# rll/rllab

Measured on NVIDIA H100. Metric: env-steps/sec (full iteration: rollout + process_samples + VPG update), higher is better.
Workload: dtype f32

## Files before the change

### rllab_b200/csrc/tile_gram.cuh

```cuda
#pragma once
#include "update_common.cuh"

namespace b200rl {

struct TileDist {
  float ls_new[3], inv_std[3], ls_old[3], inv_std_old[3], Mmu[3], var_new[3], var_new2[3], var_old[3];
  float sum_ls_new, sum_ls_old, half_log2pi_A;
};

template <class N, int MODE>
__device__ __forceinline__ void tile_dist_init(TileDist& D, const float* log_std_params, const UpdArgs& a) {
  constexpr int A = N::A;
  D.sum_ls_new = 0.f;
  D.sum_ls_old = 0.f;
#pragma unroll
  for (int k = 0; k < A; ++k) {
    D.ls_new[k] = clamp_log_std(log_std_params[k], a.log_min_std);
    const float sd = expf(D.ls_new[k]);
    D.inv_std[k] = 1.0f / sd;
    D.var_new[k] = sd * sd;
    D.var_new2[k] = 2.0f * sd * sd + 1e-8f;
    D.Mmu[k] = 2.0f / D.var_new2[k];
    D.ls_old[k] = (MODE == MODE_FVP) ? D.ls_new[k] : a.old_log_std[k];
    const float so = expf(D.ls_old[k]);
    D.inv_std_old[k] = 1.0f / so;
    D.var_old[k] = so * so;
    D.sum_ls_new += D.ls_new[k];
    D.sum_ls_old += D.ls_old[k];
  }
  D.half_log2pi_A = 0.5f * (float)A * 1.8378770664093453f;
}

template <class N, int RX, int RH1, int RH2, int RD1, int RD2, int RDM, int LD, bool PACKED = false>
struct TileGram {
  static constexpr int O = N::O, H = 32, A = N::A, TILE = 128;
  static constexpr int OQ = (O + 3) / 4;
  static_assert(N::H1 == 32 && N::H2 == 32 && A <= 3, "32-wide layers, act_dim <= 3");
  double accW1[4][4];
  double accB[OQ + 1];
  double accA;
  double accT;

  __device__ __forceinline__ void init() {
#pragma unroll
    for (int r = 0; r < 4; ++r)
#pragma unroll
      for (int c = 0; c < 4; ++c) accW1[r][c] = 0.0;
#pragma unroll
    for (int k = 0; k <= OQ; ++k) accB[k] = 0.0;
    accA = 0.0;
    accT = 0.0;
  }

  __device__ __forceinline__ void accumulate_a(const float* stage, int tid) {
    const int w1_tile = tid & 63, kh = tid >> 6;
    const int ti = w1_tile >> 3, tj = w1_tile & 7;
    const float* U = stage + (RH1 + ti) * LD + kh * 64;
    const float* V = stage + (RD2 + tj) * LD + kh * 64;
    if constexpr (PACKED) {
      float2 acc[4][4];
#pragma unroll
      for (int r = 0; r < 4; ++r)
#pragma unroll
        for (int c = 0; c < 4; ++c) acc[r][c] = make_float2(0.f, 0.f);
#pragma unroll 2
      for (int k = 0; k < 64; k += 4) {
        float4 u[4], v[4];
#pragma unroll
        for (int r = 0; r < 4; ++r) u[r] = *reinterpret_cast<const float4*>(U + r * 8 * LD + k);
#pragma unroll
        for (int c = 0; c < 4; ++c) v[c] = *reinterpret_cast<const float4*>(V + c * 8 * LD + k);
        gram_4x4(u, v, acc);
      }
#pragma unroll
      for (int r = 0; r < 4; ++r)
#pragma unroll
        for (int c = 0; c < 4; ++c) accW1[r][c] += (double)(acc[r][c].x + acc[r][c].y);
    } else {
      float acc[4][4];
#pragma unroll
      for (int r = 0; r < 4; ++r)
#pragma unroll
        for (int c = 0; c < 4; ++c) acc[r][c] = 0.f;
#pragma unroll 4
      for (int k = 0; k < 64; k += 4) {
        float4 u[4], v[4];
#pragma unroll
        for (int r = 0; r < 4; ++r) u[r] = *reinterpret_cast<const float4*>(U + r * 8 * LD + k);
#pragma unroll
        for (int c = 0; c < 4; ++c) v[c] = *reinterpret_cast<const float4*>(V + c * 8 * LD + k);
#pragma unroll
        for (int r = 0; r < 4; ++r)
#pragma unroll
          for (int c = 0; c < 4; ++c) {
            acc[r][c] = fmaf(u[r].x, v[c].x, acc[r][c]);
            acc[r][c] = fmaf(u[r].y, v[c].y, acc[r][c]);
            acc[r][c] = fmaf(u[r].z, v[c].z, acc[r][c]);
            acc[r][c] = fmaf(u[r].w, v[c].w, acc[r][c]);
          }
      }
#pragma unroll
      for (int r = 0; r < 4; ++r)
#pragma unroll
        for (int c = 0; c < 4; ++c) accW1[r][c] += (double)acc[r][c];
    }
    const int lane = tid & 31, wq = tid >> 5;
    if (wq < A) {
      const float* Hh = stage + (RH2 + lane) * LD;
      const float* M = stage + (RDM + wq) * LD;
      float s0 = 0.f, s1 = 0.f;
#pragma unroll 4
      for (int k = 0; k < TILE; k += 4) {
        const float4 hv = *reinterpret_cast<const float4*>(Hh + k);
        const float4 m = *reinterpret_cast<const float4*>(M + k);
        s0 = fmaf(hv.x, m.x, s0); s1 = fmaf(hv.y, m.y, s1);
        s0 = fmaf(hv.z, m.z, s0); s1 = fmaf(hv.w, m.w, s1);
      }
      accA += (double)(s0 + s1);
    } else if (wq == 3) {
      const float* Dr = stage + (RD2 + lane) * LD;
      float s0 = 0.f;
#pragma unroll 4
      for (int k = 0; k < TILE; k += 4) {
        const float4 d = *reinterpret_cast<const float4*>(Dr + k);
        s0 += (d.x + d.y) + (d.z + d.w);
      }
      accA += (double)s0;
    }
    if (tid < 2 * A) {
      const float* Dr = stage + (RDM + tid) * LD;
      float s0 = 0.f;
#pragma unroll 4
      for (int k = 0; k < TILE; k += 4) {
        const float4 d = *reinterpret_cast<const float4*>(Dr + k);
        s0 += (d.x + d.y) + (d.z + d.w);
      }
      accT += (double)s0;
    }
  }

  __device__ __forceinline__ void accumulate_b(const float* stage, int tid) {
    const int lane = tid & 31, wq = tid >> 5;
    const float* Dr = stage + (RD1 + lane) * LD;
    float sa[OQ + 1];
#pragma unroll
    for (int i = 0; i <= OQ; ++i) sa[i] = 0.f;
#pragma unroll 4
    for (int k = 0; k < TILE; k += 4) {
      const float4 d = *reinterpret_cast<const float4*>(Dr + k);
#pragma unroll
      for (int i = 0; i < OQ; ++i) {
        const int o = wq + 4 * i;
        if (o < O) {
          const float4 xv = *reinterpret_cast<const float4*>(stage + (RX + o) * LD + k);
          sa[i] = fmaf(xv.x, d.x, sa[i]); sa[i] = fmaf(xv.y, d.y, sa[i]);
          sa[i] = fmaf(xv.z, d.z, sa[i]); sa[i] = fmaf(xv.w, d.w, sa[i]);
        }
      }
      if (wq == 3) sa[OQ] += (d.x + d.y) + (d.z + d.w);
    }
#pragma unroll
    for (int i = 0; i <= OQ; ++i) accB[i] += (double)sa[i];
  }

  __device__ __forceinline__ void write(double* out, double* scr, int tid) {
    write(out, scr, tid, [] { __syncthreads(); });
  }
  template <class Sync>
  __device__ __forceinline__ void write(double* out, double* scr, int tid, Sync sync) {
    const int w1_tile = tid & 63, kh = tid >> 6;
    const int ti = w1_tile >> 3, tj = w1_tile & 7;
#pragma unroll
    for (int r = 0; r < 4; ++r)
#pragma unroll
      for (int c = 0; c < 4; ++c) scr[(kh * 64 + w1_tile) * 16 + r * 4 + c] = accW1[r][c];
    sync();
    if (tid < 64) {
#pragma unroll
      for (int r = 0; r < 4; ++r)
#pragma unroll
        for (int c = 0; c < 4; ++c)
          out[N::oW1 + (ti + 8 * r) * H + (tj + 8 * c)] = scr[w1_tile * 16 + r * 4 + c] + scr[(64 + w1_tile) * 16 + r * 4 + c];
    }
    const int lane = tid & 31, wq = tid >> 5;
#pragma unroll
    for (int i = 0; i < OQ; ++i) {
      const int o = wq + 4 * i;
      if (o < O) out[N::oW0 + o * H + lane] = accB[i];
    }
    if (wq == 3) {
      out[N::ob0 + lane] = accB[OQ];
      out[N::ob1 + lane] = accA;
    } else if (wq < A) {
      out[N::oWo + lane * A + wq] = accA;
    }
    if (tid < 2 * A) out[N::obo + tid] = accT;
  }
};

}
```

### rllab_b200/csrc/umma_common.cuh

```cuda
#pragma once
#include <stdint.h>

#include "update_common.cuh"

namespace b200rl {

__device__ __forceinline__ uint32_t u_smem_u32(const void* p) { return (uint32_t)__cvta_generic_to_shared(p); }
__device__ __forceinline__ float tf32_hi(float x) { return __uint_as_float(__float_as_uint(x) & 0xFFFFE000u); }

__host__ __device__ constexpr int u_kperm(int k) { return (k & ~7) | ((k & 1) << 2) | ((k >> 1) & 3); }

__device__ __forceinline__ int u_frag_row(int i, int lane) { return (lane >> 2) + 8 * ((i >> 1) & 1); }
__device__ __forceinline__ int u_frag_col(int i, int lane) { return 8 * (i >> 2) + 2 * (lane & 3) + (i & 1); }

template <int NV>
__device__ __forceinline__ void u_to_operand(const float (&f)[NV], uint32_t (&hi)[NV], uint32_t (&lo)[NV]) {
#pragma unroll
  for (int i = 0; i < NV; ++i) {
    const float v = f[(i & ~3) | ((i & 1) << 1) | ((i >> 1) & 1)];
    const float vh = tf32_hi(v);
    hi[i] = __float_as_uint(vh);
    lo[i] = __float_as_uint(v - vh);
  }
}

__device__ __forceinline__ uint64_t u_desc(uint32_t saddr, uint32_t lbo, uint32_t sbo) {
  return (uint64_t)((saddr >> 4) & 0x3FFF) | ((uint64_t)((lbo >> 4) & 0x3FFF) << 16) |
         ((uint64_t)((sbo >> 4) & 0x3FFF) << 32);
}

__device__ __forceinline__ void wg_fence() { asm volatile("wgmma.fence.sync.aligned;" ::: "memory"); }
__device__ __forceinline__ void wg_commit() { asm volatile("wgmma.commit_group.sync.aligned;" ::: "memory"); }
__device__ __forceinline__ void wg_wait_all() { asm volatile("wgmma.wait_group.sync.aligned 0;" ::: "memory"); }
template <int NV>
__device__ __forceinline__ void wg_fence_operand(float (&d)[NV]) {
#pragma unroll
  for (int i = 0; i < NV; ++i) asm volatile("" : "+f"(d[i])::"memory");
}

__device__ __forceinline__ void wg_mma_n64(float (&d)[32], uint32_t a0, uint32_t a1, uint32_t a2, uint32_t a3,
                                           uint64_t b_desc, uint32_t accumulate) {
  asm volatile(
      "{\n\t.reg .pred p;\n\tsetp.ne.b32 p, %37, 0;\n\t"
      "wgmma.mma_async.sync.aligned.m64n64k8.f32.tf32.tf32 "
      "{%0, %1, %2, %3, %4, %5, %6, %7, %8, %9, %10, %11, %12, %13, %14, %15, "
      "%16, %17, %18, %19, %20, %21, %22, %23, %24, %25, %26, %27, %28, %29, %30, %31}, "
      "{%32, %33, %34, %35}, %36, p, 1, 1;\n\t}"
      : "+f"(d[0]), "+f"(d[1]), "+f"(d[2]), "+f"(d[3]), "+f"(d[4]), "+f"(d[5]), "+f"(d[6]), "+f"(d[7]), "+f"(d[8]),
        "+f"(d[9]), "+f"(d[10]), "+f"(d[11]), "+f"(d[12]), "+f"(d[13]), "+f"(d[14]), "+f"(d[15]), "+f"(d[16]),
        "+f"(d[17]), "+f"(d[18]), "+f"(d[19]), "+f"(d[20]), "+f"(d[21]), "+f"(d[22]), "+f"(d[23]), "+f"(d[24]),
        "+f"(d[25]), "+f"(d[26]), "+f"(d[27]), "+f"(d[28]), "+f"(d[29]), "+f"(d[30]), "+f"(d[31])
      : "r"(a0), "r"(a1), "r"(a2), "r"(a3), "l"(b_desc), "r"(accumulate)
      : "memory");
}
__device__ __forceinline__ void wg_mma_n32(float (&d)[16], uint32_t a0, uint32_t a1, uint32_t a2, uint32_t a3,
                                           uint64_t b_desc, uint32_t accumulate) {
  asm volatile(
      "{\n\t.reg .pred p;\n\tsetp.ne.b32 p, %21, 0;\n\t"
      "wgmma.mma_async.sync.aligned.m64n32k8.f32.tf32.tf32 "
      "{%0, %1, %2, %3, %4, %5, %6, %7, %8, %9, %10, %11, %12, %13, %14, %15}, "
      "{%16, %17, %18, %19}, %20, p, 1, 1;\n\t}"
      : "+f"(d[0]), "+f"(d[1]), "+f"(d[2]), "+f"(d[3]), "+f"(d[4]), "+f"(d[5]), "+f"(d[6]), "+f"(d[7]), "+f"(d[8]),
        "+f"(d[9]), "+f"(d[10]), "+f"(d[11]), "+f"(d[12]), "+f"(d[13]), "+f"(d[14]), "+f"(d[15])
      : "r"(a0), "r"(a1), "r"(a2), "r"(a3), "l"(b_desc), "r"(accumulate)
      : "memory");
}

template <int NACC, int NA>
__device__ __forceinline__ void wg_split_gemm(float (&d)[NACC], const uint32_t (&ahi)[NA], const uint32_t (&alo)[NA],
                                              uint64_t b_hi, uint64_t b_lo, uint32_t kstep_bytes, int KS, bool accumulate) {
  static_assert(NACC == 32 || NACC == 16, "m64n64 or m64n32");
#pragma unroll
  for (int ks = 0; ks < NA / 4; ++ks) {
    if (ks < KS) {
      const uint64_t koff = (uint64_t)((ks * kstep_bytes) >> 4);
      const uint32_t acc0 = (accumulate || ks > 0) ? 1u : 0u;
      if constexpr (NACC == 32) {
        wg_mma_n64(d, alo[4 * ks], alo[4 * ks + 1], alo[4 * ks + 2], alo[4 * ks + 3], b_hi + koff, acc0);
        wg_mma_n64(d, ahi[4 * ks], ahi[4 * ks + 1], ahi[4 * ks + 2], ahi[4 * ks + 3], b_lo + koff, 1u);
        wg_mma_n64(d, ahi[4 * ks], ahi[4 * ks + 1], ahi[4 * ks + 2], ahi[4 * ks + 3], b_hi + koff, 1u);
      } else {
        wg_mma_n32(d, alo[4 * ks], alo[4 * ks + 1], alo[4 * ks + 2], alo[4 * ks + 3], b_hi + koff, acc0);
        wg_mma_n32(d, ahi[4 * ks], ahi[4 * ks + 1], ahi[4 * ks + 2], ahi[4 * ks + 3], b_lo + koff, 1u);
        wg_mma_n32(d, ahi[4 * ks], ahi[4 * ks + 1], ahi[4 * ks + 2], ahi[4 * ks + 3], b_hi + koff, 1u);
      }
    }
  }
}

}
```

### rllab_b200/csrc/update_umma32.cu

```cuda
#include "tile_gram.cuh"
#include "umma_common.cuh"

namespace b200rl {

constexpr int V_THREADS = 128, V_TILE = 128, V_LD = V_TILE + 4;
#ifndef B200RL_V_PACKED_GRAM
#define B200RL_V_PACKED_GRAM 1
#endif

template <class N, int MODE>
struct Umma32 {
  static constexpr int O = N::O, H = 32, A = N::A;
  static_assert(N::H1 == 32 && N::H2 == 32 && O <= 24, "tensor-core 32-wide kernel: (32,32) nets, obs_dim <= 24");
  static constexpr int KX = ((O + 7) / 8) * 8;
  static constexpr int IMG = 32 * 32 * 4, IMGX = 32 * KX * 4;
  static constexpr int o_bXT = 0, o_bW1T = o_bXT + 2 * IMGX, o_bW1 = o_bW1T + 2 * IMG,
                       o_bV1T = o_bW1 + (MODE == MODE_LOSS ? 0 : 2 * IMG),
                       o_img_end = o_bV1T + (MODE == MODE_FVP ? 2 * IMG : 0);
  static constexpr int n_small = ((64 + 2 * H * A + A + 3) / 4) * 4;
  static constexpr int o_small = o_img_end, o_stage = o_small + n_small * 4;
  static constexpr int rX = 0, rH1 = rX + O, rH2 = rH1 + H, rD1 = rH2, rD2 = rH2 + H, rDM = rD2 + H, rDL = rDM + A,
                       R = (MODE == MODE_LOSS) ? 0 : rDL + A;
  static constexpr int RR = O + (MODE == MODE_FVP ? 0 : 2 * A + 1), qX = 0, qAct = O, qOm = O + A, qAdv = O + 2 * A;
  static constexpr int w_red = ((R * V_LD * 4 + 15) / 16) * 16, w_ring = w_red + 3 * 32 * 8,
                       w_bytes = w_ring + 2 * RR * V_LD * 4;
  static constexpr int o_wg = ((o_stage + 15) / 16) * 16;
  static_assert(MODE == MODE_LOSS || 2 * 64 * 16 * 8 <= R * V_LD * 4, "stage region must hold the K-half combine scratch");
  static constexpr int NWG = (MODE == MODE_LOSS || (is_grad_mode(MODE) && A == 1)) ? 3 : 2;
  static constexpr size_t bytes = (size_t)o_wg + (size_t)NWG * w_bytes;
  static_assert(bytes <= 232448, "does not fit the 227 KB of shared memory");
};

__device__ __forceinline__ void v_wg_sync(int wg) { asm volatile("bar.sync %0, 128;" ::"r"(wg + 1) : "memory"); }

template <int K, bool IS_MAX>
__device__ __forceinline__ void v_wg_reduce_store(const double (&v)[K], double* scratch, double* out, int tid, int wg) {
  const int lane = tid & 31, warp = tid >> 5;
#pragma unroll
  for (int k = 0; k < K; ++k) {
    double s = IS_MAX ? warp_max(v[k]) : warp_sum(v[k]);
    if (lane == 0) scratch[k * 32 + warp] = s;
  }
  v_wg_sync(wg);
  if (warp == 0) {
#pragma unroll
    for (int k = 0; k < K; ++k) {
      double s = lane < 4 ? scratch[k * 32 + lane] : (IS_MAX ? -1.0e300 : 0.0);
      s = IS_MAX ? warp_max(s) : warp_sum(s);
      if (lane == 0) out[k] = s;
    }
  }
  v_wg_sync(wg);
}

template <class SMT>
__device__ __forceinline__ void v_ring_load(const UpdArgs& a, float* ring, int slot, long long tile, int tid) {
  long long s = tile * V_TILE + tid;
  if (s >= a.B) s = a.B - 1;
  float* dst = ring + (size_t)slot * SMT::RR * V_LD + tid;
#pragma unroll
  for (int q = 0; q < SMT::RR; ++q) {
    const float* src = q < SMT::qAct ? a.obs + (size_t)q * a.B + s
                       : q < SMT::qOm ? a.act + (size_t)(q - SMT::qAct) * a.B + s
                       : q < SMT::qAdv ? a.old_mean + (size_t)(q - SMT::qOm) * a.B + s
                                       : a.adv + s;
    asm volatile("cp.async.ca.shared.global [%0], [%1], 4;" ::"r"(u_smem_u32(dst + q * V_LD)), "l"(src) : "memory");
  }
  asm volatile("cp.async.commit_group;" ::: "memory");
}

__device__ __forceinline__ int v_boff(int n, int k) {
  const int kp = u_kperm(k);
  return (kp & 3) * 4 + (n & 7) * 16 + (n >> 3) * 128 + (kp >> 2) * 512;
}

template <class N, int MODE>
__global__ void __launch_bounds__(V_THREADS * Umma32<N, MODE>::NWG, 1) update_umma32_kernel(UpdArgs a) {
  using SM = Umma32<N, MODE>;
  constexpr int O = N::O, H = 32, A = N::A, P = N::P, LD = V_LD, KX = SM::KX, KSX = KX / 8;
  extern __shared__ __align__(1024) unsigned char smem[];
  float* small = reinterpret_cast<float*>(smem + SM::o_small);
  float* sb0 = small, *sb1 = small + H, *sWout = small + 2 * H, *sVout = sWout + H * A;
  float* sbo = (MODE == MODE_FVP) ? sVout + H * A : sWout + H * A;
  constexpr int NWG = SM::NWG, NT = NWG * V_THREADS;
  const int gtid = threadIdx.x, wg = gtid >> 7, tid = gtid & (V_THREADS - 1), warp = tid >> 5, lane = tid & 31, t4 = lane & 3;
  unsigned char* wreg = smem + SM::o_wg + (size_t)wg * SM::w_bytes;
  float* stage = reinterpret_cast<float*>(wreg);
  double* red_scratch = reinterpret_cast<double*>(wreg + SM::w_red);
  float* ring = reinterpret_cast<float*>(wreg + SM::w_ring);

  for (int e = gtid; e < H * H; e += NT) {
    const int i = e / H, j = e % H;
    const float w = a.params[N::oW1 + e];
    const float wh = tf32_hi(w);
    *reinterpret_cast<float*>(smem + SM::o_bW1T + v_boff(j, i)) = wh;
    *reinterpret_cast<float*>(smem + SM::o_bW1T + SM::IMG + v_boff(j, i)) = w - wh;
    if constexpr (MODE != MODE_LOSS) {
      *reinterpret_cast<float*>(smem + SM::o_bW1 + v_boff(i, j)) = wh;
      *reinterpret_cast<float*>(smem + SM::o_bW1 + SM::IMG + v_boff(i, j)) = w - wh;
    }
    if constexpr (MODE == MODE_FVP) {
      const float v = (float)a.xvec[N::oW1 + e];
      const float vh = tf32_hi(v);
      *reinterpret_cast<float*>(smem + SM::o_bV1T + v_boff(j, i)) = vh;
      *reinterpret_cast<float*>(smem + SM::o_bV1T + SM::IMG + v_boff(j, i)) = v - vh;
    }
  }
  for (int e = gtid; e < KX * H; e += NT) {
    const int o = e / H, j = e % H;
    float v = 0.f;
    if (o < O) v = (MODE == MODE_FVP) ? (float)a.xvec[N::oW0 + o * H + j] : a.params[N::oW0 + o * H + j];
    const float vh = tf32_hi(v);
    *reinterpret_cast<float*>(smem + SM::o_bXT + v_boff(j, o)) = vh;
    *reinterpret_cast<float*>(smem + SM::o_bXT + SM::IMGX + v_boff(j, o)) = v - vh;
  }
  for (int e = gtid; e < H * A; e += NT) {
    sWout[e] = a.params[N::oWo + e];
    if constexpr (MODE == MODE_FVP) sVout[e] = (float)a.xvec[N::oWo + e];
  }
  for (int e = gtid; e < H; e += NT) {
    sb0[e] = (MODE == MODE_FVP) ? (float)a.xvec[N::ob0 + e] : a.params[N::ob0 + e];
    sb1[e] = (MODE == MODE_FVP) ? (float)a.xvec[N::ob1 + e] : a.params[N::ob1 + e];
  }
  if (gtid < A) sbo[gtid] = (MODE == MODE_FVP) ? (float)a.xvec[N::obo + gtid] : a.params[N::obo + gtid];
  asm volatile("fence.proxy.async.shared::cta;" ::: "memory");
  __syncthreads();

  TileDist D;
  tile_dist_init<N, MODE>(D, a.params + N::ols, a);

  const uint64_t dXT_hi = u_desc(u_smem_u32(smem + SM::o_bXT), 512, 128), dXT_lo = u_desc(u_smem_u32(smem + SM::o_bXT + SM::IMGX), 512, 128);
  const uint64_t dW1T_hi = u_desc(u_smem_u32(smem + SM::o_bW1T), 512, 128), dW1T_lo = u_desc(u_smem_u32(smem + SM::o_bW1T + SM::IMG), 512, 128);
  const uint64_t dW1_hi = u_desc(u_smem_u32(smem + SM::o_bW1), 512, 128), dW1_lo = u_desc(u_smem_u32(smem + SM::o_bW1 + SM::IMG), 512, 128);
  const uint64_t dV1T_hi = u_desc(u_smem_u32(smem + SM::o_bV1T), 512, 128), dV1T_lo = u_desc(u_smem_u32(smem + SM::o_bV1T + SM::IMG), 512, 128);

  auto gemm2 = [&](float (&acc)[2][16], auto& f, uint64_t b_hi, uint64_t b_lo, int KS, bool accumulate) {
    constexpr int NV = sizeof(f[0]) / sizeof(float);
#pragma unroll
    for (int mb = 0; mb < 2; ++mb) {
      uint32_t hi[NV], lo[NV];
      u_to_operand(f[mb], hi, lo);
      wg_split_gemm(acc[mb], hi, lo, b_hi, b_lo, 1024, KS, accumulate);
    }
  };

  TileGram<N, SM::rX, SM::rH1, SM::rH2, SM::rD1, SM::rD2, SM::rDM, LD, B200RL_V_PACKED_GRAM != 0> gram;
  if constexpr (MODE != MODE_LOSS) gram.init();
  double s_loss = 0.0, s_kl = 0.0, m_kl = -1.0e300;

  const int ntiles = (int)n_tiles_of(a, V_TILE), nvb = gridDim.x * NWG, vb = blockIdx.x * NWG + wg;
  if (vb < ntiles) v_ring_load<SM>(a, ring, 0, tile_at(a, vb), tid);
  int slot = 0;
  for (int ti_ = vb; ti_ < ntiles; ti_ += nvb, slot ^= 1) {
    const long long tile = tile_at(a, ti_);
    asm volatile("cp.async.wait_all;" ::: "memory");
    v_wg_sync(wg);
    if (ti_ + nvb < ntiles) v_ring_load<SM>(a, ring, slot ^ 1, tile_at(a, ti_ + nvb), tid);
    const float* rs = ring + (size_t)slot * SM::RR * V_LD;
    int trow[2][2];
    long long sl[2][2];
    bool inrange[2][2], valid[2][2];
#pragma unroll
    for (int mb = 0; mb < 2; ++mb)
#pragma unroll
      for (int h = 0; h < 2; ++h) {
        trow[mb][h] = mb * 64 + warp * 16 + u_frag_row(2 * h, lane);
        const long long s = tile * V_TILE + trow[mb][h];
        inrange[mb][h] = s < a.B;
        valid[mb][h] = sample_valid(a, s);
        sl[mb][h] = inrange[mb][h] ? s : a.B - 1;
      }
    float accA[2][16], accB[2][16];
    {
      float xf[2][4 * KSX];
#pragma unroll
      for (int mb = 0; mb < 2; ++mb)
#pragma unroll
        for (int i = 0; i < 4 * KSX; ++i) {
          const int o = u_frag_col(i, lane), h = (i >> 1) & 1;
          float x = 0.f;
          if (o < O) {
            x = rs[(SM::qX + o) * LD + trow[mb][h]];
            if constexpr (MODE != MODE_LOSS) stage[(SM::rX + o) * LD + trow[mb][h]] = x;
          }
          xf[mb][i] = x;
        }
      if constexpr (MODE == MODE_FVP) {
        float h1f[2][16];
#pragma unroll
        for (int mb = 0; mb < 2; ++mb)
#pragma unroll
          for (int i = 0; i < 16; ++i) {
            const int c = u_frag_col(i, lane), h = (i >> 1) & 1;
            h1f[mb][i] = a.h_cache[(size_t)c * a.B + sl[mb][h]];
            stage[(SM::rH1 + c) * LD + trow[mb][h]] = h1f[mb][i];
          }
        wg_fence();
        gemm2(accA, xf, dXT_hi, dXT_lo, KSX, false);
        gemm2(accB, h1f, dV1T_hi, dV1T_lo, 4, false);
        wg_commit();
      } else {
        wg_fence();
        gemm2(accA, xf, dXT_hi, dXT_lo, KSX, false);
        wg_commit();
      }
    }
    wg_wait_all();
#pragma unroll
    for (int mb = 0; mb < 2; ++mb) {
      wg_fence_operand(accA[mb]);
      wg_fence_operand(accB[mb]);
    }
    {
      float v[2][16];
#pragma unroll
      for (int mb = 0; mb < 2; ++mb)
#pragma unroll
        for (int i = 0; i < 16; ++i) {
          const int c = u_frag_col(i, lane), h = (i >> 1) & 1;
          if constexpr (MODE != MODE_FVP) {
            v[mb][i] = tanh_f(accA[mb][i] + sb0[c]);
            if constexpr (is_grad_mode(MODE)) {
              stage[(SM::rH1 + c) * LD + trow[mb][h]] = v[mb][i];
              if (a.h_cache != nullptr && inrange[mb][h]) a.h_cache[(size_t)c * a.B + sl[mb][h]] = v[mb][i];
            }
          } else {
            const float h1 = stage[(SM::rH1 + c) * LD + trow[mb][h]];
            v[mb][i] = (accA[mb][i] + sb0[c]) * (1.0f - h1 * h1);
          }
        }
      wg_fence();
      gemm2(accB, v, dW1T_hi, dW1T_lo, 4, MODE == MODE_FVP);
      wg_commit();
    }
    float h2f[2][16];
    if constexpr (MODE == MODE_FVP) {
#pragma unroll
      for (int mb = 0; mb < 2; ++mb)
#pragma unroll
        for (int i = 0; i < 16; ++i)
          h2f[mb][i] = a.h_cache[(size_t)(H + u_frag_col(i, lane)) * a.B + sl[mb][(i >> 1) & 1]];
    }
    wg_wait_all();
#pragma unroll
    for (int mb = 0; mb < 2; ++mb) wg_fence_operand(accB[mb]);
    {
      float md[2][2][A];
#pragma unroll
      for (int mb = 0; mb < 2; ++mb) {
#pragma unroll
        for (int h = 0; h < 2; ++h)
#pragma unroll
          for (int k = 0; k < A; ++k) md[mb][h][k] = 0.f;
#pragma unroll
        for (int i = 0; i < 16; ++i) {
          const int c = u_frag_col(i, lane), h = (i >> 1) & 1;
          if constexpr (MODE != MODE_FVP) {
            h2f[mb][i] = tanh_f(accB[mb][i] + sb1[c]);
            if constexpr (is_grad_mode(MODE)) {
              stage[(SM::rH2 + c) * LD + trow[mb][h]] = h2f[mb][i];
              if (a.h_cache != nullptr && inrange[mb][h]) a.h_cache[(size_t)(H + c) * a.B + sl[mb][h]] = h2f[mb][i];
            }
#pragma unroll
            for (int k = 0; k < A; ++k) md[mb][h][k] = fmaf(h2f[mb][i], sWout[c * A + k], md[mb][h][k]);
          } else {
            stage[(SM::rH2 + c) * LD + trow[mb][h]] = h2f[mb][i];
            const float t2 = (accB[mb][i] + sb1[c]) * (1.0f - h2f[mb][i] * h2f[mb][i]);
#pragma unroll
            for (int k = 0; k < A; ++k)
              md[mb][h][k] = fmaf(t2, sWout[c * A + k], fmaf(h2f[mb][i], sVout[c * A + k], md[mb][h][k]));
          }
        }
      }
#pragma unroll
      for (int mb = 0; mb < 2; ++mb)
#pragma unroll
        for (int h = 0; h < 2; ++h)
#pragma unroll
          for (int k = 0; k < A; ++k) {
            md[mb][h][k] += __shfl_xor_sync(0xffffffffu, md[mb][h][k], 1);
            md[mb][h][k] += __shfl_xor_sync(0xffffffffu, md[mb][h][k], 2);
          }
      float dmu[2][2][A];
#pragma unroll
      for (int mb = 0; mb < 2; ++mb)
#pragma unroll
        for (int h = 0; h < 2; ++h) {
          const int r = trow[mb][h];
          if constexpr (MODE != MODE_FVP) {
            float act[A], om[A];
#pragma unroll
            for (int k = 0; k < A; ++k) {
              act[k] = rs[(SM::qAct + k) * LD + r];
              om[k] = rs[(SM::qOm + k) * LD + r];
            }
            const float adv_s = rs[SM::qAdv * LD + r];
            float z[A], zz[A], dmk[A], zsq = 0.f, zsq_old = 0.f, kl = 0.f;
#pragma unroll
            for (int k = 0; k < A; ++k) {
              const float mu = sbo[k] + md[mb][h][k];
              z[k] = (act[k] - mu) * D.inv_std[k];
              zz[k] = __fmul_rn(z[k], z[k]);
              zsq += zz[k];
              const float zo = (act[k] - om[k]) * D.inv_std_old[k];
              zsq_old += zo * zo;
              const float dm = om[k] - mu;
              dmk[k] = dm;
              kl += (dm * dm + D.var_old[k] - D.var_new[k]) / D.var_new2[k] + D.ls_new[k] - D.ls_old[k];
            }
            const float logp_new = -D.sum_ls_new - 0.5f * zsq - D.half_log2pi_A;
            float w_s, term;
            if (a.loss_kind == B200RL_LOSS_TRPO) {
              const float logp_old = -D.sum_ls_old - 0.5f * zsq_old - D.half_log2pi_A;
              w_s = expf(logp_new - logp_old) * adv_s;
              term = -w_s;
            } else {
              w_s = adv_s;
              term = -logp_new * adv_s;
            }
            if (!valid[mb][h]) { w_s = 0.f; term = 0.f; }
            if (t4 == 0) {
              s_loss += (double)term;
              if (valid[mb][h]) { s_kl += (double)kl; m_kl = fmax(m_kl, (double)kl); }
            }
            if constexpr (is_grad_mode(MODE)) {
#pragma unroll
              for (int k = 0; k < A; ++k) {
                dmu[mb][h][k] = -w_s * z[k] * D.inv_std[k];
                if constexpr (MODE == MODE_GRAD_KL) {
                  float dls = -w_s * (zz[k] - 1.0f);
                  if (valid[mb][h])
                    add_kl_penalty(a.penalty, dmk[k], D.var_new[k], D.var_new2[k], D.var_old[k], dmu[mb][h][k], dls);
                  if (t4 == 0) {
                    stage[(SM::rDM + k) * LD + r] = dmu[mb][h][k];
                    stage[(SM::rDL + k) * LD + r] = dls;
                  }
                } else if (t4 == 0) {
                  stage[(SM::rDM + k) * LD + r] = dmu[mb][h][k];
                  stage[(SM::rDL + k) * LD + r] = -w_s * (zz[k] - 1.0f);
                }
              }
            }
          } else {
#pragma unroll
            for (int k = 0; k < A; ++k) {
              dmu[mb][h][k] = valid[mb][h] ? (sbo[k] + md[mb][h][k]) * D.Mmu[k] : 0.f;
              if (t4 == 0) {
                stage[(SM::rDM + k) * LD + r] = dmu[mb][h][k];
                stage[(SM::rDL + k) * LD + r] = 0.f;
              }
            }
          }
        }
      if constexpr (MODE != MODE_LOSS) {
        float v[2][16];
#pragma unroll
        for (int mb = 0; mb < 2; ++mb)
#pragma unroll
          for (int i = 0; i < 16; ++i) {
            const int c = u_frag_col(i, lane), h = (i >> 1) & 1;
            float sacc = 0.f;
#pragma unroll
            for (int k = 0; k < A; ++k) sacc = fmaf(dmu[mb][h][k], sWout[c * A + k], sacc);
            v[mb][i] = sacc * (1.0f - h2f[mb][i] * h2f[mb][i]);
            stage[(SM::rD2 + c) * LD + trow[mb][h]] = v[mb][i];
          }
        wg_fence();
        gemm2(accA, v, dW1_hi, dW1_lo, 4, false);
        wg_commit();
      }
    }
    if constexpr (MODE != MODE_LOSS) {
      constexpr bool wait_first = NWG >= 3;
      if constexpr (wait_first) {
        wg_wait_all();
#pragma unroll
        for (int mb = 0; mb < 2; ++mb) wg_fence_operand(accA[mb]);
      }
      v_wg_sync(wg);
      gram.accumulate_a(stage, tid);
      v_wg_sync(wg);
      if constexpr (!wait_first) {
        wg_wait_all();
#pragma unroll
        for (int mb = 0; mb < 2; ++mb) wg_fence_operand(accA[mb]);
      }
#pragma unroll
      for (int mb = 0; mb < 2; ++mb)
#pragma unroll
        for (int i = 0; i < 16; ++i) {
          const int c = u_frag_col(i, lane), r = trow[mb][(i >> 1) & 1];
          const float h1 = stage[(SM::rH1 + c) * LD + r];
          stage[(SM::rD1 + c) * LD + r] = accA[mb][i] * (1.0f - h1 * h1);
        }
      v_wg_sync(wg);
      gram.accumulate_b(stage, tid);
      v_wg_sync(wg);
    }
  }

  if constexpr (MODE != MODE_LOSS) {
    double* out = a.partial + (size_t)vb * P;
    gram.write(out, reinterpret_cast<double*>(stage), tid, [wg] { v_wg_sync(wg); });
  }
  if constexpr (MODE != MODE_FVP) {
    double v[2] = {s_loss, s_kl};
    double mx[1] = {m_kl};
    double* sc = a.partial + (is_grad_mode(MODE) ? (size_t)nvb * P : (size_t)0) + (size_t)vb * 3;
    v_wg_reduce_store<2, false>(v, red_scratch, sc, tid, wg);
    v_wg_reduce_store<1, true>(mx, red_scratch, sc + 2, tid, wg);
  }
}

template <class N, int MODE>
static int launch_umma32(const UpdArgs& a, int* grid_out, cudaStream_t st) {
  using SM = Umma32<N, MODE>;
  B200RL_SET_MAX_SMEM((update_umma32_kernel<N, MODE>), SM::bytes);
  long long grid = num_sms();
  const long long ntiles = host_n_tiles(a, V_TILE);
  if (grid > (ntiles + SM::NWG - 1) / SM::NWG) grid = (ntiles + SM::NWG - 1) / SM::NWG;
  if (grid > MAX_PARTIAL_BLOCKS / SM::NWG) grid = MAX_PARTIAL_BLOCKS / SM::NWG;
  if (grid < 1) grid = 1;
  update_umma32_kernel<N, MODE><<<(unsigned)grid, V_THREADS * SM::NWG, SM::bytes, st>>>(a);
  B200RL_LAUNCH_CHECK("update_umma32_kernel");
  *grid_out = (int)grid * SM::NWG;
  return 0;
}

int update_umma32_launch(int mode, int obs_dim, int act_dim, const UpdArgs& a, int* grid_out, int* P_out, int* ols_out,
                         cudaStream_t st) {
  const int h1 = 32, h2 = 32;
  B200RL_DISPATCH_NET_H(32, {
    *P_out = NetT::P;
    *ols_out = NetT::ols;
    int rc = (mode == MODE_GRAD)      ? launch_umma32<NetT, MODE_GRAD>(a, grid_out, st)
             : (mode == MODE_GRAD_KL) ? launch_umma32<NetT, MODE_GRAD_KL>(a, grid_out, st)
             : (mode == MODE_LOSS)    ? launch_umma32<NetT, MODE_LOSS>(a, grid_out, st)
                                      : launch_umma32<NetT, MODE_FVP>(a, grid_out, st);
    if (rc) return rc;
  });
  return 0;
}

}
```

Before: 2.013 billion.

## Compute W1 gradient Gram via split-TF32 wgmma and register-reduced Wout grad

```diff
diff --git a/rllab_b200/csrc/tile_gram.cuh b/rllab_b200/csrc/tile_gram.cuh
--- a/rllab_b200/csrc/tile_gram.cuh
+++ b/rllab_b200/csrc/tile_gram.cuh
@@ -31,7 +31,33 @@
   D.half_log2pi_A = 0.5f * (float)A * 1.8378770664093453f;
 }
 
-template <class N, int RX, int RH1, int RH2, int RD1, int RD2, int RDM, int LD, bool PACKED = false>
+template <int O, int RX, int RD1, int LD>
+__device__ __forceinline__ void tile_gram_dw0(const float* stage, int tid, double (&acc)[(O + 3) / 4 + 1]) {
+  constexpr int OQ = (O + 3) / 4, TILE = 128;
+  const int lane = tid & 31, wq = tid >> 5;
+  const float* Dr = stage + (RD1 + lane) * LD;
+  float sa[OQ + 1];
+#pragma unroll
+  for (int i = 0; i <= OQ; ++i) sa[i] = 0.f;
+#pragma unroll 4
+  for (int k = 0; k < TILE; k += 4) {
+    const float4 d = *reinterpret_cast<const float4*>(Dr + k);
+#pragma unroll
+    for (int i = 0; i < OQ; ++i) {
+      const int o = wq + 4 * i;
+      if (o < O) {
+        const float4 xv = *reinterpret_cast<const float4*>(stage + (RX + o) * LD + k);
+        sa[i] = fmaf(xv.x, d.x, sa[i]); sa[i] = fmaf(xv.y, d.y, sa[i]);
+        sa[i] = fmaf(xv.z, d.z, sa[i]); sa[i] = fmaf(xv.w, d.w, sa[i]);
+      }
+    }
+    if (wq == 3) sa[OQ] += (d.x + d.y) + (d.z + d.w);
+  }
+#pragma unroll
+  for (int i = 0; i <= OQ; ++i) acc[i] += (double)sa[i];
+}
+
+template <class N, int RX, int RH1, int RH2, int RD1, int RD2, int RDM, int LD>
 struct TileGram {
   static constexpr int O = N::O, H = 32, A = N::A, TILE = 128;
   static constexpr int OQ = (O + 3) / 4;
@@ -57,26 +83,7 @@
     const int ti = w1_tile >> 3, tj = w1_tile & 7;
     const float* U = stage + (RH1 + ti) * LD + kh * 64;
     const float* V = stage + (RD2 + tj) * LD + kh * 64;
-    if constexpr (PACKED) {
-      float2 acc[4][4];
-#pragma unroll
-      for (int r = 0; r < 4; ++r)
-#pragma unroll
-        for (int c = 0; c < 4; ++c) acc[r][c] = make_float2(0.f, 0.f);
-#pragma unroll 2
-      for (int k = 0; k < 64; k += 4) {
-        float4 u[4], v[4];
-#pragma unroll
-        for (int r = 0; r < 4; ++r) u[r] = *reinterpret_cast<const float4*>(U + r * 8 * LD + k);
-#pragma unroll
-        for (int c = 0; c < 4; ++c) v[c] = *reinterpret_cast<const float4*>(V + c * 8 * LD + k);
-        gram_4x4(u, v, acc);
-      }
-#pragma unroll
-      for (int r = 0; r < 4; ++r)
-#pragma unroll
-        for (int c = 0; c < 4; ++c) accW1[r][c] += (double)(acc[r][c].x + acc[r][c].y);
-    } else {
+    {
       float acc[4][4];
 #pragma unroll
       for (int r = 0; r < 4; ++r)
@@ -140,27 +147,7 @@
   }
 
   __device__ __forceinline__ void accumulate_b(const float* stage, int tid) {
-    const int lane = tid & 31, wq = tid >> 5;
-    const float* Dr = stage + (RD1 + lane) * LD;
-    float sa[OQ + 1];
-#pragma unroll
-    for (int i = 0; i <= OQ; ++i) sa[i] = 0.f;
-#pragma unroll 4
-    for (int k = 0; k < TILE; k += 4) {
-      const float4 d = *reinterpret_cast<const float4*>(Dr + k);
-#pragma unroll
-      for (int i = 0; i < OQ; ++i) {
-        const int o = wq + 4 * i;
-        if (o < O) {
-          const float4 xv = *reinterpret_cast<const float4*>(stage + (RX + o) * LD + k);
-          sa[i] = fmaf(xv.x, d.x, sa[i]); sa[i] = fmaf(xv.y, d.y, sa[i]);
-          sa[i] = fmaf(xv.z, d.z, sa[i]); sa[i] = fmaf(xv.w, d.w, sa[i]);
-        }
-      }
-      if (wq == 3) sa[OQ] += (d.x + d.y) + (d.z + d.w);
-    }
-#pragma unroll
-    for (int i = 0; i <= OQ; ++i) accB[i] += (double)sa[i];
+    tile_gram_dw0<O, RX, RD1, LD>(stage, tid, accB);
   }
 
   __device__ __forceinline__ void write(double* out, double* scr, int tid) {
diff --git a/rllab_b200/csrc/umma_common.cuh b/rllab_b200/csrc/umma_common.cuh
--- a/rllab_b200/csrc/umma_common.cuh
+++ b/rllab_b200/csrc/umma_common.cuh
@@ -7,6 +7,8 @@
 
 __device__ __forceinline__ uint32_t u_smem_u32(const void* p) { return (uint32_t)__cvta_generic_to_shared(p); }
 __device__ __forceinline__ float tf32_hi(float x) { return __uint_as_float(__float_as_uint(x) & 0xFFFFE000u); }
+
+__device__ __forceinline__ float tf32_rn(float x) { return __uint_as_float((__float_as_uint(x) + 0x1000u) & 0xFFFFE000u); }
 
 __host__ __device__ constexpr int u_kperm(int k) { return (k & ~7) | ((k & 1) << 2) | ((k >> 1) & 3); }
 
@@ -32,6 +34,8 @@
 __device__ __forceinline__ void wg_fence() { asm volatile("wgmma.fence.sync.aligned;" ::: "memory"); }
 __device__ __forceinline__ void wg_commit() { asm volatile("wgmma.commit_group.sync.aligned;" ::: "memory"); }
 __device__ __forceinline__ void wg_wait_all() { asm volatile("wgmma.wait_group.sync.aligned 0;" ::: "memory"); }
+template <int N>
+__device__ __forceinline__ void wg_wait() { asm volatile("wgmma.wait_group.sync.aligned %0;" ::"n"(N) : "memory"); }
 template <int NV>
 __device__ __forceinline__ void wg_fence_operand(float (&d)[NV]) {
 #pragma unroll
diff --git a/rllab_b200/csrc/update_umma32.cu b/rllab_b200/csrc/update_umma32.cu
--- a/rllab_b200/csrc/update_umma32.cu
+++ b/rllab_b200/csrc/update_umma32.cu
@@ -4,9 +4,6 @@
 namespace b200rl {
 
 constexpr int V_THREADS = 128, V_TILE = 128, V_LD = V_TILE + 4;
-#ifndef B200RL_V_PACKED_GRAM
-#define B200RL_V_PACKED_GRAM 1
-#endif
 
 template <class N, int MODE>
 struct Umma32 {
@@ -19,13 +16,16 @@
                        o_img_end = o_bV1T + (MODE == MODE_FVP ? 2 * IMG : 0);
   static constexpr int n_small = ((64 + 2 * H * A + A + 3) / 4) * 4;
   static constexpr int o_small = o_img_end, o_stage = o_small + n_small * 4;
-  static constexpr int rX = 0, rH1 = rX + O, rH2 = rH1 + H, rD1 = rH2, rD2 = rH2 + H, rDM = rD2 + H, rDL = rDM + A,
-                       R = (MODE == MODE_LOSS) ? 0 : rDL + A;
+  static constexpr int GIMG = 32 * V_TILE * 4;
+  static constexpr int rX = 0, rH1 = rX + O, rDM = rH1 + H, rDL = rDM + A, rG = ((rDL + A + 7) / 8) * 8, rD1 = rG,
+                       R = (MODE == MODE_LOSS) ? 0 : rG;
+  static_assert(32 * V_LD * 4 <= 2 * GIMG, "D1 rows fit in the D2 image");
   static constexpr int RR = O + (MODE == MODE_FVP ? 0 : 2 * A + 1), qX = 0, qAct = O, qOm = O + A, qAdv = O + 2 * A;
-  static constexpr int w_red = ((R * V_LD * 4 + 15) / 16) * 16, w_ring = w_red + 3 * 32 * 8,
-                       w_bytes = w_ring + 2 * RR * V_LD * 4;
-  static constexpr int o_wg = ((o_stage + 15) / 16) * 16;
-  static_assert(MODE == MODE_LOSS || 2 * 64 * 16 * 8 <= R * V_LD * 4, "stage region must hold the K-half combine scratch");
+  static constexpr int AL = (MODE == MODE_LOSS) ? 16 : 128;
+  static constexpr int w_red = ((R * V_LD * 4 + (MODE == MODE_LOSS ? 0 : 2 * GIMG) + 15) / 16) * 16,
+                       w_ring = w_red + 3 * 32 * 8, w_bytes = ((w_ring + 2 * RR * V_LD * 4 + AL - 1) / AL) * AL;
+  static constexpr int o_wg = ((o_stage + AL - 1) / AL) * AL;
+  static_assert(MODE == MODE_LOSS || 3 * 64 * A * 8 <= R * V_LD * 4, "stage rows must hold the final reduction scratch");
   static constexpr int NWG = (MODE == MODE_LOSS || (is_grad_mode(MODE) && A == 1)) ? 3 : 2;
   static constexpr size_t bytes = (size_t)o_wg + (size_t)NWG * w_bytes;
   static_assert(bytes <= 232448, "does not fit the 227 KB of shared memory");
@@ -67,6 +67,11 @@
     asm volatile("cp.async.ca.shared.global [%0], [%1], 4;" ::"r"(u_smem_u32(dst + q * V_LD)), "l"(src) : "memory");
   }
   asm volatile("cp.async.commit_group;" ::: "memory");
+}
+
+__device__ __forceinline__ int v_wo_col(int lane) {
+  const int g = lane >> 2;
+  return 8 * (g >> 1) + 2 * (lane & 3) + (g & 1);
 }
 
 __device__ __forceinline__ int v_boff(int n, int k) {
@@ -144,8 +149,22 @@
     }
   };
 
-  TileGram<N, SM::rX, SM::rH1, SM::rH2, SM::rD1, SM::rD2, SM::rDM, LD, B200RL_V_PACKED_GRAM != 0> gram;
-  if constexpr (MODE != MODE_LOSS) gram.init();
+  constexpr int OQ = (O + 3) / 4;
+  double gW1[16];
+  double gW0[OQ + 1];
+  double gWo[A];
+  double gT;
+  if constexpr (MODE != MODE_LOSS) {
+#pragma unroll
+    for (int i = 0; i < 16; ++i) gW1[i] = 0.0;
+#pragma unroll
+    for (int i = 0; i <= OQ; ++i) gW0[i] = 0.0;
+#pragma unroll
+    for (int k = 0; k < A; ++k) gWo[k] = 0.0;
+#pragma unroll
+    gT = 0.0;
+  }
+  unsigned char* gimg = reinterpret_cast<unsigned char*>(stage + SM::rG * LD);
   double s_loss = 0.0, s_kl = 0.0, m_kl = -1.0e300;
 
   const int ntiles = (int)n_tiles_of(a, V_TILE), nvb = gridDim.x * NWG, vb = blockIdx.x * NWG + wg;
@@ -234,6 +253,7 @@
       wg_commit();
     }
     float h2f[2][16];
+    float pwo[8][A];
     if constexpr (MODE == MODE_FVP) {
 #pragma unroll
       for (int mb = 0; mb < 2; ++mb)
@@ -258,13 +278,11 @@
           if constexpr (MODE != MODE_FVP) {
             h2f[mb][i] = tanh_f(accB[mb][i] + sb1[c]);
             if constexpr (is_grad_mode(MODE)) {
-              stage[(SM::rH2 + c) * LD + trow[mb][h]] = h2f[mb][i];
               if (a.h_cache != nullptr && inrange[mb][h]) a.h_cache[(size_t)(H + c) * a.B + sl[mb][h]] = h2f[mb][i];
             }
 #pragma unroll
             for (int k = 0; k < A; ++k) md[mb][h][k] = fmaf(h2f[mb][i], sWout[c * A + k], md[mb][h][k]);
           } else {
-            stage[(SM::rH2 + c) * LD + trow[mb][h]] = h2f[mb][i];
             const float t2 = (accB[mb][i] + sb1[c]) * (1.0f - h2f[mb][i] * h2f[mb][i]);
 #pragma unroll
             for (int k = 0; k < A; ++k)
@@ -327,17 +345,14 @@
 #pragma unroll
               for (int k = 0; k < A; ++k) {
                 dmu[mb][h][k] = -w_s * z[k] * D.inv_std[k];
+                float dls = -w_s * (zz[k] - 1.0f);
                 if constexpr (MODE == MODE_GRAD_KL) {
-                  float dls = -w_s * (zz[k] - 1.0f);
                   if (valid[mb][h])
                     add_kl_penalty(a.penalty, dmk[k], D.var_new[k], D.var_new2[k], D.var_old[k], dmu[mb][h][k], dls);
-                  if (t4 == 0) {
-                    stage[(SM::rDM + k) * LD + r] = dmu[mb][h][k];
-                    stage[(SM::rDL + k) * LD + r] = dls;
-                  }
-                } else if (t4 == 0) {
+                }
+                if (t4 == 0) {
                   stage[(SM::rDM + k) * LD + r] = dmu[mb][h][k];
-                  stage[(SM::rDL + k) * LD + r] = -w_s * (zz[k] - 1.0f);
+                  stage[(SM::rDL + k) * LD + r] = dls;
                 }
               }
             }
@@ -355,15 +370,25 @@
       if constexpr (MODE != MODE_LOSS) {
         float v[2][16];
 #pragma unroll
+        for (int q = 0; q < 8; ++q)
+#pragma unroll
+          for (int k = 0; k < A; ++k) pwo[q][k] = 0.f;
+#pragma unroll
         for (int mb = 0; mb < 2; ++mb)
 #pragma unroll
           for (int i = 0; i < 16; ++i) {
-            const int c = u_frag_col(i, lane), h = (i >> 1) & 1;
+            const int c = u_frag_col(i, lane), h = (i >> 1) & 1, q = 2 * (i >> 2) + (i & 1);
             float sacc = 0.f;
 #pragma unroll
-            for (int k = 0; k < A; ++k) sacc = fmaf(dmu[mb][h][k], sWout[c * A + k], sacc);
+            for (int k = 0; k < A; ++k) {
+              sacc = fmaf(dmu[mb][h][k], sWout[c * A + k], sacc);
+              pwo[q][k] = fmaf(h2f[mb][i], dmu[mb][h][k], pwo[q][k]);
+            }
             v[mb][i] = sacc * (1.0f - h2f[mb][i] * h2f[mb][i]);
-            stage[(SM::rD2 + c) * LD + trow[mb][h]] = v[mb][i];
+            const int s = trow[mb][h], off = (s & 3) * 4 + (c & 7) * 16 + (c >> 3) * 128 + (s >> 2) * 512;
+            const float vh = tf32_rn(v[mb][i]);
+            *reinterpret_cast<float*>(gimg + off) = vh;
+            *reinterpret_cast<float*>(gimg + SM::GIMG + off) = v[mb][i] - vh;
           }
         wg_fence();
         gemm2(accA, v, dW1_hi, dW1_lo, 4, false);
@@ -371,20 +396,78 @@
       }
     }
     if constexpr (MODE != MODE_LOSS) {
-      constexpr bool wait_first = NWG >= 3;
-      if constexpr (wait_first) {
+      asm volatile("fence.proxy.async.shared::cta;" ::: "memory");
+      v_wg_sync(wg);
+      float accG[16];
+      if constexpr (NWG >= 3) {
         wg_wait_all();
 #pragma unroll
         for (int mb = 0; mb < 2; ++mb) wg_fence_operand(accA[mb]);
       }
+#pragma unroll
+      for (int k = 0; k < A; ++k) {
+        float kept = 0.f;
+#pragma unroll
+        for (int q = 0; q < 8; ++q) {
+          float p = pwo[q][k];
+          p += __shfl_xor_sync(0xffffffffu, p, 4);
+          p += __shfl_xor_sync(0xffffffffu, p, 8);
+          p += __shfl_xor_sync(0xffffffffu, p, 16);
+          if (q == (lane >> 2)) kept = p;
+        }
+        gWo[k] += (double)kept;
+      }
+      {
+        constexpr int V_GC = 2;
+        const uint64_t dG_hi = u_desc(u_smem_u32(gimg), 512, 128), dG_lo = u_desc(u_smem_u32(gimg + SM::GIMG), 512, 128);
+        const float* h1r = stage + (SM::rH1 + 16 * warp + (lane >> 2)) * LD + t4;
+#pragma unroll
+        for (int cg = 0; cg < 16 / V_GC; ++cg) {
+          uint32_t hi[4 * V_GC], lo[4 * V_GC];
+#pragma unroll
+          for (int ks = 0; ks < V_GC; ++ks)
+#pragma unroll
+            for (int e = 0; e < 4; ++e) {
+              float x = 0.f;
+              if (warp < 2) x = h1r[(e & 1) * 8 * LD + 8 * (cg * V_GC + ks) + 4 * (e >> 1)];
+              const float xh = tf32_rn(x);
+              hi[4 * ks + e] = __float_as_uint(xh);
+              lo[4 * ks + e] = __float_as_uint(x - xh);
+            }
+          const uint64_t koff = (uint64_t)((cg * V_GC * 1024) >> 4);
+          wg_fence();
+          wg_split_gemm(accG, hi, lo, dG_hi + koff, dG_lo + koff, 1024, V_GC, cg > 0);
+          wg_commit();
+          if (cg > 0) wg_wait<1>();
+        }
+      }
+      if (warp == 3 || tid < 2 * A) {
+        const unsigned char* gr = gimg + (lane & 7) * 16 + (lane >> 3) * 128;
+        const float* Dr = stage + (SM::rDM + tid) * LD;
+        float s0 = 0.f;
+#pragma unroll 4
+        for (int k = 0; k < V_TILE; k += 4) {
+          float4 d;
+          if (warp == 3) {
+            const float4 dh = *reinterpret_cast<const float4*>(gr + k * 128);
+            const float4 dl = *reinterpret_cast<const float4*>(gr + SM::GIMG + k * 128);
+            d = make_float4(dh.x + dl.x, dh.y + dl.y, dh.z + dl.z, dh.w + dl.w);
+          } else {
+            d = *reinterpret_cast<const float4*>(Dr + k);
+          }
+          s0 += (d.x + d.y) + (d.z + d.w);
+        }
+        gT += (double)s0;
+      }
+      wg_wait_all();
+#pragma unroll
+      for (int mb = 0; mb < 2; ++mb) wg_fence_operand(accA[mb]);
+      wg_fence_operand(accG);
+      if (warp < 2) {
+#pragma unroll
+        for (int i = 0; i < 16; ++i) gW1[i] += (double)accG[i];
+      }
       v_wg_sync(wg);
-      gram.accumulate_a(stage, tid);
-      v_wg_sync(wg);
-      if constexpr (!wait_first) {
-        wg_wait_all();
-#pragma unroll
-        for (int mb = 0; mb < 2; ++mb) wg_fence_operand(accA[mb]);
-      }
 #pragma unroll
       for (int mb = 0; mb < 2; ++mb)
 #pragma unroll
@@ -394,14 +477,37 @@
           stage[(SM::rD1 + c) * LD + r] = accA[mb][i] * (1.0f - h1 * h1);
         }
       v_wg_sync(wg);
-      gram.accumulate_b(stage, tid);
+      tile_gram_dw0<O, SM::rX, SM::rD1, LD>(stage, tid, gW0);
       v_wg_sync(wg);
     }
   }
 
   if constexpr (MODE != MODE_LOSS) {
     double* out = a.partial + (size_t)vb * P;
-    gram.write(out, reinterpret_cast<double*>(stage), tid, [wg] { v_wg_sync(wg); });
+#pragma unroll
+    for (int i = 0; i < 16; ++i) {
+      const int row = 16 * warp + u_frag_row(i, lane), col = u_frag_col(i, lane);
+      if (warp < 2) out[N::oW1 + row * H + col] = gW1[i];
+    }
+#pragma unroll
+    for (int q = 0; q < OQ; ++q) {
+      const int o = warp + 4 * q;
+      if (o < O) out[N::oW0 + o * H + lane] = gW0[q];
+    }
+    if (warp == 3) {
+      out[N::ob0 + lane] = gW0[OQ];
+      out[N::ob1 + lane] = gT;
+    }
+    if (tid < 2 * A) out[N::obo + tid] = gT;
+    double* scr = reinterpret_cast<double*>(stage);
+#pragma unroll
+    for (int k = 0; k < A; ++k) scr[k * 128 + tid] = gWo[k];
+    v_wg_sync(wg);
+    if (tid < 32 * A) {
+      const int k = tid >> 5;
+      const double* sk = scr + k * 128 + lane;
+      out[N::oWo + v_wo_col(lane) * A + k] = ((sk[0] + sk[32]) + sk[64]) + sk[96];
+    }
   }
   if constexpr (MODE != MODE_FVP) {
     double v[2] = {s_loss, s_kl};
```

Result: faster. 2.174 billion, median of 6 (+8.0%).
